# ymxlzgy/echoscene

Measured on AMD Instinct MI355X. Metric: denoising steps/sec (layout+SDF) for 32-node scene-graph, 64^3 SDF (3x16^3 latent), full step = one DDPM layout step + one DDIM shape step over all objects; `value` = the FUSED step (both loops as one hipGraph per step, the layout step on a parallel branch: what the K timed steps ran); `full_steps_p, higher is better.
Workload: dtype f16 MFMA operands / f32 accumulate (shape UNet); f32 (layout, GCN)

## Files before the change

### echoscene_amd/csrc/es_vol.hip

```cpp
#include "es_common.h"
#include <string>
#include <algorithm>
#include <cstdlib>
#include <mutex>
#include <type_traits>

namespace {

__device__ __forceinline__ int f_swz(int row) { return (0x1320 >> (((row >> 2) & 3) * 4)) & 3; }

constexpr int GN_VT = 64;

__global__ __launch_bounds__(256) void k_gn_partial(const es_gn_args a, float* part, int vt) {
    __shared__ float ssum4[4][2048], ssq4[4][2048];
    float* ssum = ssum4[0];
    float* ssq = ssq4[0];
    const int o = blockIdx.y, tile = blockIdx.x, C = a.C1 + a.C2;
    const int v0 = tile * vt;
    const int nv = min(vt, a.V - v0);
    const int c4n = C >> 2;
    const int CX = 64;
    const int cx = threadIdx.x & (CX - 1), vy = threadIdx.x >> 6;
    for (int c4 = cx; c4 < c4n; c4 += CX) {
        const int c = c4 * 4;
// ... 1578 lines not shown
    f4 fin[MI2][7];
#pragma unroll
    for (int i2 = 0; i2 < MI2; ++i2)
#pragma unroll
        for (int j = 0; j < 7; ++j) {
            const int i = strm * MI2 + i2;
            f4 v = ((const f4*)smem)[(long)(0 * NCH_ + hh) * (PART_FLOATS / 4) + (i * 7 + j) * 64 + lane];
#pragma unroll
            for (int s = 1; s < KS_; ++s) v += ((const f4*)smem)[(long)(s * NCH_ + hh) * (PART_FLOATS / 4) + (i * 7 + j) * 64 + lane];
            fin[i2][j] = v;
        }
    asm volatile("s_waitcnt lgkmcnt(0)" ::: "memory");
    if constexpr (NCH_ == 1) conv_epilogue<64, 8, true, true, EPI_>(a, g, fin, smem, M, m0, by * BN + half0 * 112, 2 * wave, lane, S, bz, ncdhw);
    else conv_epilogue<64, 4, true, true, EPI_>(a, g, fin, smem, M, m0, by * BN, wave, lane, S, bz, ncdhw);
}

template <int EPI_, int NS_ = 3>
__global__ __launch_bounds__(768, 3) void k_linear_ws(const es_conv_args a, const ConvGeom g, int ncb) {
    constexpr int BM_ = 256, NC_ = 8, NP_ = 4, NS = NS_;
    constexpr int WROWS = BM_ / (NC_ / 2), MI = WROWS / 16;
    constexpr int A_BYTES = BM_ * BK * 2, B_BYTES = BNP * BK * 2, STAGE_BYTES = A_BYTES + B_BYTES, RING_BYTES = NS * STAGE_BYTES;
    constexpr int NA = (BM_ / 16) / NP_, NB = (BNP / 16) / NP_, NLOAD = NA + NB;
    constexpr unsigned OOB = 0x80000000u;
    typedef __attribute__((address_space(3))) void* lds_ptr;
    extern __shared__ __attribute__((aligned(16))) char smem[];
    const int tid = threadIdx.x, lane = tid & 63;
    const int wave = __builtin_amdgcn_readfirstlane(tid >> 6);
    const long M = (long)g.O * g.D * g.H * g.W;
#ifdef ES_STAMP
    unsigned long long* stamp = g_stamp_buf ? g_stamp_buf + ((size_t)(blockIdx.x + gridDim.x * blockIdx.y) * (NC_ + NP_) + wave) * 8 : nullptr;
#endif
    ES_STAMP_AT(0);
    int bx, byg;
    {
        const int gx = gridDim.x, gy = gridDim.y, nwg = gx * gy;
        const int orig = blockIdx.x + gx * blockIdx.y;
        const int xcd = orig & 7, q = nwg >> 3, r = nwg & 7;
        const int L = (xcd < r ? xcd * (q + 1) : r * (q + 1) + (xcd - r) * q) + (orig >> 3);
        const long slab = (long)a.Cin * BN * 2 * ncb;
        int npanel = (int)(((long)gy * slab + (3L << 20) - 1) / (3L << 20));
        npanel = npanel < 1 ? 1 : (npanel > gy ? gy : npanel);
        const int Pw = (gy + npanel - 1) / npanel, full = gx * Pw;
        const int p = L / full, rr = L - p * full;
        const int w = (gy - p * Pw) < Pw ? (gy - p * Pw) : Pw;
        bx = rr / w;
        byg = p * Pw + (rr - bx * w);
    }
    const long m0 = (long)bx * BM_;
    const int by0 = byg * ncb;
    const int kch = a.Cin >> 5;
    const int total = kch * ncb;
    if (wave >= NC_) {
        const int pw = wave - NC_;
        unsigned voff[NA];
#pragma unroll
        for (int j = 0; j < NA; ++j) {
            const int p = (pw + NP_ * j) * 64 + lane;
            const int row = p >> 2;
            const long m = m0 + row;
            voff[j] = m < M ? (unsigned)(m * a.Cin * 2 + (((p & 3) ^ f_swz(row)) * 16)) : OOB;
        }
        const __amdgpu_buffer_rsrc_t rA = __builtin_amdgcn_make_buffer_rsrc(uniform_ptr(a.a), (short)0, (int)OOB, 0x00020000);
        const _Float16* Wg = (const _Float16*)a.w;
        int cb = 0, c = 0, islot = 0;
        __amdgpu_buffer_rsrc_t rB = __builtin_amdgcn_make_buffer_rsrc(uniform_ptr(Wg + (long)by0 * kch * (BNP * BK)), (short)0, (int)OOB, 0x00020000);
        const unsigned voffB = (unsigned)lane * 16u;
        auto issue = [&]() __attribute__((always_inline)) {
            char* dst = smem + __builtin_amdgcn_readfirstlane(islot) * STAGE_BYTES;
            const unsigned sA = (unsigned)__builtin_amdgcn_readfirstlane(c) * 64u;
            const unsigned sB = (unsigned)__builtin_amdgcn_readfirstlane(c) * (unsigned)B_BYTES;
#pragma unroll
            for (int j = 0; j < NA; ++j)
                __builtin_amdgcn_raw_ptr_buffer_load_lds(rA, (lds_ptr)(dst + (pw + NP_ * j) * 1024), 16, (int)voff[j], (int)sA, 0, 0);
#pragma unroll
            for (int j = 0; j < NB; ++j) {
                const int q = pw + NP_ * j;
                const unsigned vB = q * 16 >= BN ? OOB : voffB;
                __builtin_amdgcn_raw_ptr_buffer_load_lds(rB, (lds_ptr)(dst + A_BYTES + q * 1024), 16, (int)vB, (int)(sB + (unsigned)q * 1024u), 0, 0);
            }
            islot = islot == NS - 1 ? 0 : islot + 1;
            if (++c == kch) {
                c = 0; ++cb;
                rB = __builtin_amdgcn_make_buffer_rsrc(uniform_ptr(Wg + (long)(by0 + cb) * kch * (BNP * BK)), (short)0, (int)OOB, 0x00020000);
            }
        };
        issue();
        if (total > 1) issue();
        if (NS == 4 && total > 2) issue();
        for (int u = 0; u < total; ++u) {
            const int ahead = total - 1 - u < NS - 2 ? total - 1 - u : NS - 2;
            if (ahead >= 2) wait_vmcnt<2 * NLOAD>(); else if (ahead == 1) wait_vmcnt<NLOAD>(); else wait_vmcnt<0>();
            __builtin_amdgcn_s_barrier();
            if (u + NS - 1 < total) issue();
        }
        return;
    }
    const int wm = wave >> 1, wn = wave & 1;
    const int i16 = lane & 15, q = lane >> 4;
    const int fragA = (wm * WROWS + i16) * 64 + ((q ^ f_swz(i16)) << 4);
    const int fragB = A_BYTES + (wn * 112 + i16) * 64 + ((q ^ f_swz(i16)) << 4);
    int slot = 0;
    for (int cb = 0; cb < ncb; ++cb) {
        f4 acc[MI][7];
#pragma unroll
        for (int i = 0; i < MI; ++i)
#pragma unroll
            for (int j = 0; j < 7; ++j) acc[i][j] = f4{0.f, 0.f, 0.f, 0.f};
        h8 af[MI], bfr[7];
        __builtin_amdgcn_s_barrier();
        ws_read_frags<MI>(smem + slot * STAGE_BYTES, fragA, fragB, af, bfr);
        slot = slot == NS - 1 ? 0 : slot + 1;
        for (int ks = 0; ks + 1 < kch; ++ks) {
            const char* const An = smem + slot * STAGE_BYTES;
            slot = slot == NS - 1 ? 0 : slot + 1;
#pragma unroll
            for (int j = 0; j < 7; ++j) acc[0][j] = __builtin_amdgcn_mfma_f32_16x16x32_f16(af[0], bfr[j], acc[0][j], 0, 0, 0);
            __builtin_amdgcn_sched_barrier(0);
            asm volatile("s_waitcnt lgkmcnt(0)" ::: "memory");
            __builtin_amdgcn_s_barrier();
            __builtin_amdgcn_sched_barrier(0);
#pragma unroll
            for (int i = 1; i < MI; ++i) {
                af[i - 1] = *(const h8*)(An + fragA + (i - 1) * 1024);
                __builtin_amdgcn_sched_barrier(0);
                if (i < MI - 1) {
#pragma unroll
                    for (int j = 0; j < 7; ++j) acc[i][j] = __builtin_amdgcn_mfma_f32_16x16x32_f16(af[i], bfr[j], acc[i][j], 0, 0, 0);
                    __builtin_amdgcn_sched_barrier(0);
                } else {
#pragma unroll
                    for (int j = 0; j < 7; ++j) {
                        acc[i][j] = __builtin_amdgcn_mfma_f32_16x16x32_f16(af[i], bfr[j], acc[i][j], 0, 0, 0);
                        __builtin_amdgcn_sched_barrier(0);
                        bfr[j] = *(const h8*)(An + fragB + j * 1024);
                        __builtin_amdgcn_sched_barrier(0);
                    }
                }
            }
            af[MI - 1] = *(const h8*)(An + fragA + (MI - 1) * 1024);
            __builtin_amdgcn_sched_barrier(0);
        }
        ws_mma<MI>(acc, af, bfr);
#ifdef ES_STAMP
        if (cb < 3) ES_STAMP_AT(1 + 2 * cb);
#endif
        conv_epilogue<BM_, NC_, true, true, EPI_, true>(a, g, acc, smem + RING_BYTES, M, m0, (by0 + cb) * BN, wave, lane, 1, 0, 0);
#ifdef ES_STAMP
        if (cb < 3) ES_STAMP_AT(2 + 2 * cb);
#endif
    }
}

constexpr int AT_K = 64;

template <int DP, int NWV, int NRT, int MINW = (DP <= 64 ? 3 : 2)>
__global__ __launch_bounds__(64 * NWV, MINW) void k_attention(const es_attn_args a) {
    constexpr int AT_Q = 16 * NRT * NWV;
    constexpr int KLD = DP + 8;
    __shared__ __attribute__((aligned(16))) _Float16 Ks[AT_K * KLD];
    __shared__ __attribute__((aligned(16))) _Float16 Vs[AT_K * KLD];
    const int tid = threadIdx.x, lane = tid & 63, wave = tid >> 6;
    const int i16 = lane & 15, q4 = lane >> 4;
    const int nx = gridDim.x, nwg = nx * (int)gridDim.y;
    const int orig = blockIdx.x + nx * blockIdx.y;
    const int xcd = orig & 7, xq = nwg >> 3, xr = nwg & 7;
    const int L = (xcd < xr ? xcd * (xq + 1) : xr * (xq + 1) + (xcd - xr) * xq) + (orig >> 3);
    const int bh = L / nx, rtile = L - bh * nx;
    const int b = bh / a.heads, h = bh - b * a.heads;
    const int C = a.heads * a.dhead, ldq = 3 * C;
    const _Float16* base = (const _Float16*)a.qkv + (long)b * a.Ntok * ldq + h * a.dhead;
    const int q0 = rtile * AT_Q + wave * (16 * NRT);

    h8 qf[NRT][DP / 32];
#pragma unroll
    for (int rt = 0; rt < NRT; ++rt)
#pragma unroll
        for (int kc = 0; kc < DP / 32; ++kc) {
            const int d0 = kc * 32 + q4 * 8, row = q0 + rt * 16 + i16;
            const _Float16* p = base + (long)row * ldq + d0;
#pragma unroll
            for (int e = 0; e < 8; ++e) qf[rt][kc][e] = (d0 + e < a.dhead && row < a.Ntok) ? p[e] : (_Float16)0.f;
        }
    f4 oacc[NRT][DP / 16];
    float mrow[NRT], lrow[NRT];
#pragma unroll
    for (int rt = 0; rt < NRT; ++rt) {
        mrow[rt] = -INFINITY; lrow[rt] = 0.f;
#pragma unroll
        for (int j = 0; j < DP / 16; ++j) oacc[rt][j] = f4{0.f, 0.f, 0.f, 0.f};
    }

    constexpr int NT = 64 * NWV, CPR = DP / 4, NITEM = AT_K * CPR, NIT = (NITEM + NT - 1) / NT;
    constexpr bool PREFETCH = DP <= 96;
    h4 kreg[NIT], vreg[NIT];
    unsigned kvoff[NIT];
#pragma unroll
    for (int it = 0; it < NIT; ++it) {
        const int idx = tid + it * NT;
        const int key = idx / CPR, d = (idx - key * CPR) * 4;
        kvoff[it] = (idx < NITEM && d < a.dhead) ? (unsigned)(key * ldq + d) * 2u : 0x80000000u;
    }
    const int nrec = (int)(((long)(a.Ntok - 1) * ldq + a.dhead) * 2);
    const __amdgpu_buffer_rsrc_t rK = __builtin_amdgcn_make_buffer_rsrc(uniform_ptr(base + C), (short)0, nrec, 0x00020000);
    const __amdgpu_buffer_rsrc_t rV = __builtin_amdgcn_make_buffer_rsrc(uniform_ptr(base + 2 * C), (short)0, nrec, 0x00020000);
    auto gload = [&](int k0) __attribute__((always_inline)) {
        const unsigned koff = (unsigned)k0 * (unsigned)ldq * 2u;
#pragma unroll
        for (int it = 0; it < NIT; ++it) {
            kreg[it] = __builtin_bit_cast(h4, __builtin_amdgcn_raw_buffer_load_b64(rK, (int)(kvoff[it] + koff), 0, 0));
            vreg[it] = __builtin_bit_cast(h4, __builtin_amdgcn_raw_buffer_load_b64(rV, (int)(kvoff[it] + koff), 0, 0));
        }
    };
    if (PREFETCH) gload(0);
    for (int k0 = 0; k0 < a.Ntok; k0 += AT_K) {
        __syncthreads();
#pragma unroll
        for (int it = 0; it < NIT; ++it) {
            const int idx = tid + it * NT;
            if (idx < NITEM) {
                const int key = idx / CPR, d = (idx - key * CPR) * 4;
                h4 kv = kreg[PREFETCH ? it : 0], vv = vreg[PREFETCH ? it : 0];
                if (!PREFETCH) {
                    kv = h4{0, 0, 0, 0}; vv = h4{0, 0, 0, 0};
                    if (d < a.dhead && k0 + key < a.Ntok) {
                        const _Float16* p = base + (long)(k0 + key) * ldq + d;
                        kv = *(const h4*)(p + C);
                        vv = *(const h4*)(p + 2 * C);
                    }
                }
                *(h4*)&Ks[key * KLD + d] = kv;
                *(h4*)&Vs[key * KLD + d] = vv;
            }
        }
        __syncthreads();
        if (PREFETCH && k0 + AT_K < a.Ntok) gload(k0 + AT_K);
        f4 s[NRT][4];
#pragma unroll
        for (int rt = 0; rt < NRT; ++rt)
#pragma unroll
            for (int t = 0; t < 4; ++t) s[rt][t] = f4{0.f, 0.f, 0.f, 0.f};
#pragma unroll
        for (int t = 0; t < 4; ++t)
#pragma unroll
            for (int kc = 0; kc < DP / 32; ++kc) {
                const h8 kf = *(const h8*)&Ks[(t * 16 + i16) * KLD + kc * 32 + q4 * 8];
#pragma unroll
                for (int rt = 0; rt < NRT; ++rt) s[rt][t] = __builtin_amdgcn_mfma_f32_16x16x32_f16(kf, qf[rt][kc], s[rt][t], 0, 0, 0);
            }
        h8 pf[NRT][2];
        typedef float f2 __attribute__((ext_vector_type(2)));
        const float c2 = a.scale * 1.44269504088896340736f;
        if (k0 + AT_K > a.Ntok) {
            asm volatile("" ::: "memory");
#pragma unroll
            for (int rt = 0; rt < NRT; ++rt)
#pragma unroll
                for (int t = 0; t < 4; ++t)
#pragma unroll
                    for (int r = 0; r < 4; ++r) {
                        float v = k0 + t * 16 + q4 * 4 + r >= a.Ntok ? -INFINITY : s[rt][t][r];
                        asm volatile("" : "+v"(v));
                        s[rt][t][r] = v;
                    }
        }
#pragma unroll
        for (int rt = 0; rt < NRT; ++rt) {
            float mx = -INFINITY;
#pragma unroll
            for (int t = 0; t < 4; ++t)
#pragma unroll
                for (int r = 0; r < 4; ++r) mx = fmaxf(mx, s[rt][t][r]);
            {
                float e, o;
                es_pair16(mx, e, o); mx = fmaxf(e, o);
                es_pair32(mx, e, o); mx = fmaxf(e, o);
            }
            const float mnew = fmaxf(mrow[rt], mx * c2);
            const float alpha = __builtin_amdgcn_exp2f(mrow[rt] - mnew);
            const f2 c22 = {c2, c2}, nm2 = {-mnew, -mnew};
            f2 ps2 = {0.f, 0.f};
#pragma unroll
            for (int t = 0; t < 4; ++t)
#pragma unroll
                for (int hf = 0; hf < 2; ++hf) {
                    const f2 v = {s[rt][t][2 * hf], s[rt][t][2 * hf + 1]};
                    const f2 e = __builtin_elementwise_fma(v, c22, nm2);
                    const f2 pp = {__builtin_amdgcn_exp2f(e[0]), __builtin_amdgcn_exp2f(e[1])};
                    ps2 += pp;
                    pf[rt][t >> 1][(t & 1) * 4 + 2 * hf] = (_Float16)pp[0];
                    pf[rt][t >> 1][(t & 1) * 4 + 2 * hf + 1] = (_Float16)pp[1];
                }
            float ps = ps2[0] + ps2[1];
            {
                float e, o;
                es_pair16(ps, e, o); ps = e + o;
                es_pair32(ps, e, o); ps = e + o;
            }
            lrow[rt] = lrow[rt] * alpha + ps;
            mrow[rt] = mnew;
            if (__ballot(alpha != 1.0f) != 0) {
                const f2 al2 = {alpha, alpha};
#pragma unroll
                for (int j = 0; j < DP / 16; ++j) {
                    f2 lo = {oacc[rt][j][0], oacc[rt][j][1]}, hi = {oacc[rt][j][2], oacc[rt][j][3]};
                    lo *= al2; hi *= al2;
                    oacc[rt][j] = f4{lo[0], lo[1], hi[0], hi[1]};
                }
            }
        }
#pragma unroll
        for (int kc = 0; kc < AT_K / 32; ++kc)
#pragma unroll
            for (int j = 0; j < DP / 16; ++j) {
                typedef short s4v __attribute__((ext_vector_type(4)));
                typedef __attribute__((address_space(3))) s4v* lds_s4;
                const _Float16* vp = &Vs[(kc * 32 + q4 * 4 + (i16 >> 2)) * KLD + j * 16 + (i16 & 3) * 4];
                const h4 v0 = __builtin_bit_cast(h4, __builtin_amdgcn_ds_read_tr16_b64_v4i16((lds_s4)vp));
                const h4 v1 = __builtin_bit_cast(h4, __builtin_amdgcn_ds_read_tr16_b64_v4i16((lds_s4)(vp + 16 * KLD)));
                const h8 vf = {v0[0], v0[1], v0[2], v0[3], v1[0], v1[1], v1[2], v1[3]};
#pragma unroll
                for (int rt = 0; rt < NRT; ++rt) oacc[rt][j] = __builtin_amdgcn_mfma_f32_16x16x32_f16(vf, pf[rt][kc], oacc[rt][j], 0, 0, 0);
            }
    }
    _Float16* out = (_Float16*)a.out_f16 + (long)b * a.Ntok * C + h * a.dhead;
#pragma unroll
    for (int rt = 0; rt < NRT; ++rt) {
        const int row = q0 + rt * 16 + i16;
        if (row >= a.Ntok) continue;
        const float inv = 1.0f / lrow[rt];
#pragma unroll
        for (int j = 0; j < DP / 16; ++j) {
            const int d = j * 16 + q4 * 4;
            if (d < a.dhead) {
                const f4 o = oacc[rt][j] * inv;
                const h4 hv = {(_Float16)o[0], (_Float16)o[1], (_Float16)o[2], (_Float16)o[3]};
                *(h4*)&out[(long)row * C + d] = hv;
            }
        }
    }
}

__global__ __launch_bounds__(256) void k_conv_small_n(const es_conv_args a, const ConvGeom g, int ncdhw) {
    extern __shared__ __attribute__((aligned(16))) char smem[];
    _Float16* wl = (_Float16*)smem;
    const int wn = a.N * 27 * a.Cin;
    for (int i = threadIdx.x * 8; i < wn; i += 256 * 8) *(h8*)(wl + i) = *(const h8*)((const _Float16*)a.w + i);
    __syncthreads();
    const long M = (long)g.O * g.D * g.H * g.W;
    const long m = (long)blockIdx.x * 256 + threadIdx.x;
    if (m >= M) return;
    const int w_ = (int)(m & (g.W - 1)), h_ = (int)((m >> g.lw) & (g.H - 1)), d_ = (int)((m >> (g.lw + g.lh)) & (g.D - 1));
    const long o = m >> (g.lw + g.lh + g.ld);
    float acc[4] = {0.f, 0.f, 0.f, 0.f};
    const _Float16* A = (const _Float16*)a.a;
    for (int tap = 0; tap < 27; ++tap) {
        const int id = d_ + tap / 9 - 1, ih = h_ + (tap / 3) % 3 - 1, iw = w_ + tap % 3 - 1;
        if (id < 0 || id >= g.D || ih < 0 || ih >= g.H || iw < 0 || iw >= g.W) continue;
        const _Float16* src = A + (((o * g.D + id) * g.H + ih) * g.W + iw) * a.Cin;
        for (int c = 0; c < a.Cin; c += 8) {
            const h8 x = *(const h8*)(src + c);
#pragma unroll
            for (int n = 0; n < 4; ++n) {
                if (n < a.N) {
                    const h8 wv = *(const h8*)(wl + (n * 27 + tap) * a.Cin + c);
#pragma unroll
                    for (int e = 0; e < 8; ++e) acc[n] += (float)x[e] * (float)wv[e];
                }
            }
        }
    }
    const long V = (long)g.D * g.H * g.W;
    for (int n = 0; n < a.N; ++n) {
        float v = acc[n] + (a.bias ? a.bias[n] : 0.f);
        if (ncdhw) a.out_f32[(o * a.N + n) * V + (m - o * V)] = v;
        else a.out_f32[m * a.out_ld + n] = v;
    }
}

__global__ __launch_bounds__(256) void k_conv_small_n_tiled(const es_conv_args a, const ConvGeom g, int ncdhw) {
    extern __shared__ __attribute__((aligned(16))) char smem[];
    const int Cin = a.Cin, c8n = Cin >> 3, vstride = Cin * 2 + 16;
    char* xt = smem;
    _Float16* wl = (_Float16*)(smem + 1000 * vstride);
    const int wn = a.N * 27 * Cin;
    for (int i = threadIdx.x * 8; i < wn; i += 256 * 8) *(h8*)(wl + i) = *(const h8*)((const _Float16*)a.w + i);
    const int tw = g.W >> 3, th = g.H >> 3, td = g.D >> 3;
    int t = blockIdx.x;
    const int bw = t % tw; t /= tw;
    const int bh = t % th; t /= th;
    const int bd = t % td;
    const long o = t / td;
    const _Float16* A = (const _Float16*)a.a + o * (long)g.D * g.H * g.W * Cin;
    for (int i = threadIdx.x; i < 1000 * c8n; i += 256) {
        const int c8 = i % c8n, v = i / c8n;
        const int lw = v % 10, lh = (v / 10) % 10, ld_ = v / 100;
        const int iw = bw * 8 + lw - 1, ih = bh * 8 + lh - 1, id = bd * 8 + ld_ - 1;
        h8 x = {0, 0, 0, 0, 0, 0, 0, 0};
        if (iw >= 0 && iw < g.W && ih >= 0 && ih < g.H && id >= 0 && id < g.D)
            x = *(const h8*)(A + (((long)id * g.H + ih) * g.W + iw) * Cin + c8 * 8);
        *(h8*)(xt + v * vstride + c8 * 16) = x;
    }
    __syncthreads();
    typedef _Float16 h2v __attribute__((ext_vector_type(2)));
    float acc[2][4] = {{0.f, 0.f, 0.f, 0.f}, {0.f, 0.f, 0.f, 0.f}};
    const int lw = threadIdx.x & 7, lh = (threadIdx.x >> 3) & 7, ld0 = threadIdx.x >> 6;
    for (int tap = 0; tap < 27; ++tap) {
        const int kd = tap / 9, kh = (tap / 3) % 3, kw = tap % 3;
        const char* p0 = xt + (((ld0 + kd) * 10 + lh + kh) * 10 + lw + kw) * vstride;
        const char* p1 = p0 + 400 * vstride;
        for (int c8 = 0; c8 < c8n; ++c8) {
            const h8 x0 = *(const h8*)(p0 + c8 * 16), x1 = *(const h8*)(p1 + c8 * 16);
#pragma unroll
            for (int n = 0; n < 4; ++n) {
                if (n < a.N) {
                    const h8 wv = *(const h8*)(wl + (n * 27 + tap) * Cin + c8 * 8);
#pragma unroll
                    for (int e = 0; e < 4; ++e) {
                        const h2v w2 = {wv[2 * e], wv[2 * e + 1]};
                        acc[0][n] = __builtin_amdgcn_fdot2(h2v{x0[2 * e], x0[2 * e + 1]}, w2, acc[0][n], false);
                        acc[1][n] = __builtin_amdgcn_fdot2(h2v{x1[2 * e], x1[2 * e + 1]}, w2, acc[1][n], false);
                    }
                }
            }
        }
    }
    const long V = (long)g.D * g.H * g.W;
#pragma unroll
    for (int k = 0; k < 2; ++k) {
        const long vox = (((long)(bd * 8 + ld0 + 4 * k) * g.H) + bh * 8 + lh) * g.W + bw * 8 + lw;
        for (int n = 0; n < a.N; ++n) {
            const float v = acc[k][n] + (a.bias ? a.bias[n] : 0.f);
            if (ncdhw) a.out_f32[(o * a.N + n) * V + vox] = v;
            else a.out_f32[(o * V + vox) * a.out_ld + n] = v;
        }
    }
}

constexpr int N16_ROWS = 6 * 6 * 18;
constexpr int N16_A_BYTES = 44 * 1024, N16_B_BYTES = 28 * 1024;

__global__ __launch_bounds__(256, 2) void k_conv_n16(const es_conv_args a, const ConvGeom g) {
    typedef __attribute__((address_space(3))) void* lds_ptr;
    constexpr unsigned OOB = 0x80000000u;
    extern __shared__ __attribute__((aligned(16))) char smem[];
    char* As = smem;
    char* Bs = smem + N16_A_BYTES;
    const int tid = threadIdx.x, lane = tid & 63;
    const int wave = __builtin_amdgcn_readfirstlane(tid >> 6);
    const int tw = g.W >> 4, th = g.H >> 2, td = g.D >> 2;
    int t = blockIdx.x;
    const int bw = t % tw; t /= tw;
    const int bh = t % th; t /= th;
    const int bd = t % td;
    const int o = t / td;
    const int Cin = a.Cin, kch = Cin >> 5;
    constexpr int NPA = 11, NPB = 7;
    unsigned voff[NPA];
#pragma unroll
    for (int j = 0; j < NPA; ++j) {
        const int piece = wave + 4 * j;
        const int slot = piece * 64 + lane;
        const int row = slot >> 2;
        const int lc = (slot & 3) ^ f_swz(row);
        const int hw = row % 18, hh = (row / 18) % 6, hd = row / 108;
        const int d = bd * 4 - 1 + hd, h = bh * 4 - 1 + hh, w = bw * 16 - 1 + hw;
        const bool ok = row < N16_ROWS && d >= 0 && d < g.D && h >= 0 && h < g.H && w >= 0 && w < g.W;
        voff[j] = ok ? (unsigned)((((o * g.D + d) * g.H + h) * g.W + w) * Cin * 2 + lc * 16) : OOB;
    }
    const __amdgpu_buffer_rsrc_t rA = __builtin_amdgcn_make_buffer_rsrc(uniform_ptr(a.a), (short)0, (int)OOB, 0x00020000);
    const __amdgpu_buffer_rsrc_t rB = __builtin_amdgcn_make_buffer_rsrc(uniform_ptr(a.w), (short)0, (int)OOB, 0x00020000);
    const int i16 = lane & 15, q = lane >> 4;
    const int rowbase = (wave * 6) * 18 + i16;
    f4 acc[4];
#pragma unroll
    for (int i = 0; i < 4; ++i) acc[i] = f4{0.f, 0.f, 0.f, 0.f};
// ... 678 lines not shown
        const int np = vo("conv_st_np");
        const dim3 grid((unsigned)((M + st_bm - 1) / st_bm), ntn, S);
        const bool stt = want_stats && epi_stats;
        int rc = 1;
        const int ns = vo("conv_st_ns");
        if (st_bm == 64 && np == 4 && ns == 3) rc = launch_ws<64, 4, 4, 3>(a, g, ncdhw, grid, st, upm, geglu, stt);
        else if (st_bm == 64 && np == 4 && ns == 6) rc = launch_ws<64, 4, 4, 6>(a, g, ncdhw, grid, st, upm, geglu, stt);
        else if (st_bm == 128 && np == 4 && ns == 3) rc = launch_ws<128, 4, 4, 3>(a, g, ncdhw, grid, st, upm, geglu, stt);
        else if (st_bm == 128 && np == 8 && ns == 3) rc = launch_ws<128, 4, 8, 3>(a, g, ncdhw, grid, st, upm, geglu, stt);
        else if (st_bm == 128 && np == 8 && ns == 5) rc = launch_ws<128, 4, 8, 5>(a, g, ncdhw, grid, st, upm, geglu, stt);
        else ES_REQUIRE(false, "es_conv_mfma_f16: conv_st_bm=%d conv_st_np=%d conv_st_ns=%d is not a built tile", st_bm, np, ns);
        if (rc) return rc;
        stats_done = stt;
    } else if (deep) {
        S = 1;
        hipLaunchKernelGGL(k_linear_deep, dim3((unsigned)((M + 63) / 64), ntn, 1), dim3(256), 7 * (64 * BK * 2 + BNP * BK * 2), st, *a, g);
    } else if (route256) {
        dim3 grid((unsigned)((M + 255) / 256), ntn, S);
        if (ncb > 1) {
            const dim3 lgrid(grid.x, (unsigned)(ntn / ncb), 1);
            constexpr int LDSLIN = LDS256 + 8 * 16 * 116 * 4;
            static const char* ring_env = getenv("ES_LIN_RING");
            if (geglu && ring_env && atoi(ring_env) == 4) hipLaunchKernelGGL((k_linear_ws<ES_EPI_GEGLU, 4>), lgrid, dim3(768), LDSLIN_GEGLU, st, *a, g, ncb);
            else if (geglu) hipLaunchKernelGGL((k_linear_ws<ES_EPI_GEGLU>), lgrid, dim3(768), LDSLIN, st, *a, g, ncb);
            else hipLaunchKernelGGL((k_linear_ws<ES_EPI_NONE>), lgrid, dim3(768), LDSLIN, st, *a, g, ncb);
        } else if (ws && (!geglu || !upm)) {
            static const char* ns_env = getenv("ES_CONV_NS");
            const int ns = ns_env ? atoi(ns_env) : 3;
            const bool stt = want_stats && epi_stats;
            static const char* a3_env = getenv("ES_CONV_A3");
            const bool a3 = (a3_env ? atoi(a3_env) != 0 : ES_CONV_A3_DEFAULT) && a->taps == 27 && a->mode == ES_CONV_SAME && !a->a2 && a->W <= 16 && a->W >= 4;
            if (a3) {
                static std::once_flag once3;
                static hipError_t err3 = hipSuccess;
                std::call_once(once3, [] {
                    err3 = hipFuncSetAttribute((const void*)k_conv_ws3<false>, hipFuncAttributeMaxDynamicSharedMemorySize, 6 * 16384);
                    for (auto fl : {std::pair<const void*, int>{(const void*)k_conv_ws3<true>, 6 * 16384}, {(const void*)k_conv_ws3<false, true>, 9 * 16384},
                                    {(const void*)k_conv_ws3<true, true>, 9 * 16384}}) {
                        const hipError_t e2 = hipFuncSetAttribute(fl.first, hipFuncAttributeMaxDynamicSharedMemorySize, fl.second);
                        if (err3 == hipSuccess) err3 = e2;
                    }
                });
                static const char* gb_env = getenv("ES_CONV_GB");
                ES_REQUIRE(err3 == hipSuccess, "es_conv_mfma_f16: hipFuncSetAttribute failed: %s", hipGetErrorString(err3));
                if (!gb_env || atoi(gb_env) != 0) {
                    if (stt) hipLaunchKernelGGL((k_conv_ws3<true, true>), grid, dim3(768), 9 * 16384, st, *a, g);
                    else hipLaunchKernelGGL((k_conv_ws3<false, true>), grid, dim3(768), 9 * 16384, st, *a, g);
                }
                else if (stt) hipLaunchKernelGGL((k_conv_ws3<true>), grid, dim3(768), 6 * 16384, st, *a, g);
                else hipLaunchKernelGGL((k_conv_ws3<false>), grid, dim3(768), 6 * 16384, st, *a, g);
                if (stt) stats_done = true;
            } else {
            int rc;
            if (ns == 4) rc = launch_ws<256, 8, 4, 4>(a, g, ncdhw, grid, st, upm, geglu, stt);
            else if (ns == 5) rc = launch_ws<256, 8, 4, 5>(a, g, ncdhw, grid, st, upm, geglu, stt);
            else rc = launch_ws<256, 8, 4, 3>(a, g, ncdhw, grid, st, upm, geglu, stt);
            if (rc) return rc;
            if (stt) stats_done = true;
            }
        }
        else if (upm) hipLaunchKernelGGL((k_conv_lean<256, 8, true>), grid, dim3(512), LDS256, st, *a, g, ncdhw);
        else hipLaunchKernelGGL((k_conv_lean<256, 8>), grid, dim3(512), LDS256, st, *a, g, ncdhw);
    } else if ((wg128 >= 512 || S > 1) && !tiny_split) {
        dim3 grid((unsigned)((M + 127) / 128), ntn, S);
        if (upm) hipLaunchKernelGGL((k_conv_lean<128, 4, true>), grid, dim3(256), LDS128, st, *a, g, ncdhw);
        else hipLaunchKernelGGL((k_conv_lean<128, 4>), grid, dim3(256), LDS128, st, *a, g, ncdhw);
    } else {
        dim3 grid((unsigned)((M + 63) / 64), ntn, tiny_split ? S : 1);
        if (upm) hipLaunchKernelGGL((k_conv_lean<64, 4, true>), grid, dim3(256), LDS64, st, *a, g, ncdhw);
        else hipLaunchKernelGGL((k_conv_lean<64, 4>), grid, dim3(256), LDS64, st, *a, g, ncdhw);
    }
    if (S > 1) {
        const long n4 = M * (a->N / 4);
        const int blocks = (int)((n4 + 255) / 256 < 4096 ? (n4 + 255) / 256 : 4096);
        if (a->gn_part_out && part_ok) {
            const int V = a->D * a->H * a->W;
            const int vt = gn_voxel_tile(Oh, V);
            hipLaunchKernelGGL(k_conv_splitk_reduce_gn, dim3((V + vt - 1) / vt, a->O), dim3(256), 0, st, *a, M, V, S, vt);
        } else
            hipLaunchKernelGGL(k_conv_splitk_reduce, dim3(blocks), dim3(256), 0, st, *a, M, a->D * a->H * a->W, S);
    }
    if (want_stats && !stats_done) {
        ES_REQUIRE(a->out_f32, "es_conv_mfma_f16: this launch's route forms gn_stats_out by a pass over the fp32 output: out_f32 must be given "
                               "(es_conv_emits_gn_stats() == 0)");
        const long n4 = ((M + 63) / 64) * (a->N / 4);
        const int blocks = (int)((n4 + 255) / 256 < 8192 ? (n4 + 255) / 256 : 8192);
        hipLaunchKernelGGL(k_rowgroup_stats, dim3(blocks), dim3(256), 0, st, (const float*)a->out_f32, M, a->N, a->out_ld, a->gn_stats_out);
    }
    ES_CHECK_HIP(hipGetLastError());
    return 0;
}

extern "C" int es_conv_mfma_f16(const es_conv_args* a, es_stream stream) { return conv_dispatch(a, stream, nullptr); }

extern "C" int es_conv_emits_gn_stats(const es_conv_args* a) {
    int e = 0;
    return conv_dispatch(a, nullptr, &e) == 0 ? (e & 1) : -1;
}

extern "C" int es_conv_emits_gn_part(const es_conv_args* a) {
    int e = 0;
    return conv_dispatch(a, nullptr, &e) == 0 ? ((e >> 1) & 1) : -1;
}

extern "C" int es_conv_split_of(const es_conv_args* a) {
    int e = 0;
    return conv_dispatch(a, nullptr, &e) == 0 ? (e >> 8) : -1;
}

extern "C" int es_groupnorm_vol(const es_gn_args* a, es_stream stream) {
    const int C = a->C1 + a->C2;
    ES_REQUIRE(C % a->groups == 0 && C <= 2048 && a->groups <= 64, "es_groupnorm_vol: C=%d groups=%d", C, a->groups);
    ES_REQUIRE(a->C1 % 8 == 0 && a->C2 % 8 == 0, "es_groupnorm_vol: channel counts must be multiples of 8 (%d,%d)", a->C1, a->C2);
    ES_REQUIRE(a->stats != nullptr, "es_groupnorm_vol: stats scratch missing");
    const long Oh = a->O_hint < 0 ? -(long)a->O_hint : (long)(a->O_hint > a->O ? a->O_hint : a->O);
    const int vt = gn_voxel_tile(Oh, a->V);
    const int ntiles = (a->V + vt - 1) / vt;
    float* part = a->stats;
    const bool from_rg = a->stats1 && (!a->x2 || a->stats2) && a->V % 64 == 0 && (a->x1_is_f16 || vo("gn_rg") != 0);
    ES_REQUIRE(!a->x1_is_f16 || (from_rg && !a->x2 && !a->raw_f16),
               "es_groupnorm_vol: an f16 source needs the producer's row-group sums (stats1), one source, no raw copy");
    ES_REQUIRE(!a->part_in || (!from_rg && !a->x2), "es_groupnorm_vol: part_in needs one source and no row-group sums");
    if (a->part_in) part = (float*)a->part_in;
    else if (!from_rg) hipLaunchKernelGGL(k_gn_partial, dim3(ntiles, a->O), dim3(256), 0, (hipStream_t)stream, *a, part, vt);
    int vpb = 32;
    while (vpb > 8 && (long)a->O * ((a->V + vpb - 1) / vpb) < 512) vpb >>= 1;
    while (vpb < 1024 && (long)a->O * ((a->V + vpb - 1) / vpb) > 16384) vpb <<= 1;
    const float* fin = nullptr;
    if (from_rg) {
        hipLaunchKernelGGL(k_gn_finalize_rg, dim3(a->groups, a->O), dim3(256), 0, (hipStream_t)stream, *a, part);
        fin = part;
    } else if (ntiles > 128) {
        float* f = a->part_in ? a->stats : part + (size_t)a->O * ntiles * a->groups * 2;
        hipLaunchKernelGGL(k_gn_finalize, dim3(a->groups, a->O), dim3(256), 0, (hipStream_t)stream, *a, part, ntiles, f);
        fin = f;
    }
    hipLaunchKernelGGL(k_gn_apply, dim3((a->V + vpb - 1) / vpb, a->O), dim3(256), 0, (hipStream_t)stream, *a, part, ntiles, vpb, fin);
    ES_CHECK_HIP(hipGetLastError());
    return 0;
}

extern "C" int es_layernorm_tokens(const es_ln_args* a, es_stream stream) {
    ES_REQUIRE(a->C <= 1024 && a->C > 0 && a->C % 4 == 0, "es_layernorm_tokens: C=%d (a multiple of 4, max 1024)", a->C);
    long wgs = ((long)a->M + 3) / 4;
    if (wgs > 2048) wgs = 2048;
    hipLaunchKernelGGL(k_layernorm, dim3((unsigned)wgs), dim3(256), 0, (hipStream_t)stream, *a);
    ES_CHECK_HIP(hipGetLastError());
    return 0;
}

extern "C" int es_attention_f16(const es_attn_args* a, es_stream stream) {
    ES_REQUIRE(a->dhead % 4 == 0 && a->dhead <= 256 && a->dhead > 0, "es_attention_f16: dhead=%d (multiple of 4, <= 256)", a->dhead);
    ES_REQUIRE(a->scale > 0.f, "es_attention_f16: scale=%g must be positive (the row maximum is taken over the raw scores)", (double)a->scale);
    const bool big = a->Ntok >= 512 && a->dhead <= 96;
    const int rows = big ? 128 : 64;
    dim3 grid((a->Ntok + rows - 1) / rows, a->B * a->heads);
    hipStream_t st = (hipStream_t)stream;
    if (a->dhead <= 32) { if (big) hipLaunchKernelGGL((k_attention<32, 4, 2>), grid, dim3(256), 0, st, *a); else hipLaunchKernelGGL((k_attention<32, 4, 1>), grid, dim3(256), 0, st, *a); }
    else if (a->dhead <= 64) { if (big) hipLaunchKernelGGL((k_attention<64, 4, 2>), grid, dim3(256), 0, st, *a); else hipLaunchKernelGGL((k_attention<64, 4, 1>), grid, dim3(256), 0, st, *a); }
    else if (a->dhead <= 96) { if (big) hipLaunchKernelGGL((k_attention<96, 4, 2>), grid, dim3(256), 0, st, *a); else hipLaunchKernelGGL((k_attention<96, 4, 1>), grid, dim3(256), 0, st, *a); }
    else hipLaunchKernelGGL((k_attention<256, 4, 1>), grid, dim3(256), 0, st, *a);
    ES_CHECK_HIP(hipGetLastError());
    return 0;
}

extern "C" int es_geglu_f16(const es_geglu_args* a, es_stream stream) {
    ES_REQUIRE(a->C4 % 4 == 0, "es_geglu_f16: C4=%d", a->C4);
    const long n4 = (long)a->M * (a->C4 / 4);
    const int blocks = (int)((n4 + 255) / 256 < 8192 ? (n4 + 255) / 256 : 8192);
    hipLaunchKernelGGL(k_geglu, dim3(blocks), dim3(256), 0, (hipStream_t)stream, *a);
    ES_CHECK_HIP(hipGetLastError());
    return 0;
}

static int latent_to_cl(const float* x, int O, int C, int V, int Cpad, void* out, int is_f32, es_stream stream) {
    const long n = (long)O * V * Cpad;
    const int blocks = (int)((n + 255) / 256 < 4096 ? (n + 255) / 256 : 4096);
    hipLaunchKernelGGL(k_to_cl, dim3(blocks), dim3(256), 0, (hipStream_t)stream, x, O, C, V, Cpad, (_Float16*)out, is_f32);
    ES_CHECK_HIP(hipGetLastError());
    return 0;
}
extern "C" int es_latent_to_cl_f16(const float* x, int O, int C, int V, int Cpad, void* out, es_stream stream) { return latent_to_cl(x, O, C, V, Cpad, out, 0, stream); }
extern "C" int es_latent_to_cl_f32(const float* x, int O, int C, int V, int Cpad, void* out, es_stream stream) { return latent_to_cl(x, O, C, V, Cpad, out, 1, stream); }

extern "C" int es_split_f16x3(const float* x, long M, int C, void* out, es_stream stream) {
    ES_REQUIRE(x && out && M > 0 && C > 0 && C % 4 == 0, "es_split_f16x3: M=%ld C=%d (C a multiple of 4)", M, C);
    const long n = M * (C / 4);
    const int blocks = (int)((n + 255) / 256 < 8192 ? (n + 255) / 256 : 8192);
    hipLaunchKernelGGL(k_split_f16x3, dim3(blocks), dim3(256), 0, (hipStream_t)stream, x, M, C, (_Float16*)out);
    ES_CHECK_HIP(hipGetLastError());
    return 0;
}

extern "C" int es_shape_stem(const es_stem_args* a, es_stream stream) {
    const long n1 = (long)a->O * 32 * 512, n2 = (long)a->O * 512;
    const int Cx = a->Cin ? a->Cin : 3;
    ES_REQUIRE(Cx >= 1 && Cx <= 4, "es_shape_stem: Cin=%d (3 or 4)", Cx);
    (void)n1;
    hipLaunchKernelGGL(k_stem1, dim3(64, a->O), dim3(256), (size_t)(Cx * 288 + 32 * Cx * 27) * 4, (hipStream_t)stream, *a);
    {
        static std::once_flag once_s;
        static hipError_t attr_s = hipSuccess;
        std::call_once(once_s, [] { attr_s = hipFuncSetAttribute((const void*)k_stem2, hipFuncAttributeMaxDynamicSharedMemorySize, 32 * 513 * 4); });
        ES_REQUIRE(attr_s == hipSuccess, "es_shape_stem: hipFuncSetAttribute failed: %s", hipGetErrorString(attr_s));
    }
    hipLaunchKernelGGL(k_stem2, dim3((unsigned)((n2 * 8 + 255) / 256)), dim3(256), 32 * 513 * 4, (hipStream_t)stream, *a);
    ES_CHECK_HIP(hipGetLastError());
    return 0;
}

extern "C" int es_vq_lookup(const es_vq_args* a, es_stream stream) {
    ES_REQUIRE(a->n_embed > 0 && a->n_embed * 16 <= 160 * 1024 - 1024, "es_vq_lookup: n_embed=%d too large for LDS", a->n_embed);
    ES_REQUIRE(a->Cpad >= 3, "es_vq_lookup: Cpad=%d", a->Cpad);
    {
        static std::once_flag once;
        static hipError_t attr_err = hipSuccess;
        std::call_once(once, [] {
            attr_err = hipFuncSetAttribute((const void*)k_vq_lookup, hipFuncAttributeMaxDynamicSharedMemorySize, 160 * 1024 - 1024);
        });
        ES_REQUIRE(attr_err == hipSuccess, "es_vq_lookup: hipFuncSetAttribute failed: %s", hipGetErrorString(attr_err));
    }
    const long M = (long)a->O * a->V;
    hipLaunchKernelGGL(k_vq_lookup, dim3((unsigned)((M + 255) / 256)), dim3(256), (size_t)a->n_embed * 16, (hipStream_t)stream, *a);
    ES_CHECK_HIP(hipGetLastError());
    return 0;
}
```

Measured before the change: 55.84.

## Defer softmax rescale with threshold, fold row-sum into PV MFMA, split ragged tile

```diff
diff --git a/echoscene_amd/csrc/es_vol.hip b/echoscene_amd/csrc/es_vol.hip
--- a/echoscene_amd/csrc/es_vol.hip
+++ b/echoscene_amd/csrc/es_vol.hip
@@ -1754,8 +1754,9 @@
 }
 
 constexpr int AT_K = 64;
-
-template <int DP, int NWV, int NRT, int MINW = (DP <= 64 ? 3 : 2)>
+constexpr float AT_TAU = 8.f;
+
+template <int DP, int NWV, int NRT, bool LSUM, int MINW = (DP <= 64 ? 3 : 2)>
 __global__ __launch_bounds__(64 * NWV, MINW) void k_attention(const es_attn_args a) {
     constexpr int AT_Q = 16 * NRT * NWV;
     constexpr int KLD = DP + 8;
@@ -1796,12 +1797,15 @@
     constexpr bool PREFETCH = DP <= 96;
     h4 kreg[NIT], vreg[NIT];
     unsigned kvoff[NIT];
+    int vsoff[NIT];
 #pragma unroll
     for (int it = 0; it < NIT; ++it) {
         const int idx = tid + it * NT;
         const int key = idx / CPR, d = (idx - key * CPR) * 4;
         kvoff[it] = (idx < NITEM && d < a.dhead) ? (unsigned)(key * ldq + d) * 2u : 0x80000000u;
-    }
+        vsoff[it] = key * KLD + ((LSUM && d == a.dhead) ? DP : d);
+    }
+    if (LSUM && tid < AT_K) *(h4*)&Vs[tid * KLD + a.dhead] = h4{(_Float16)1.f, (_Float16)0.f, (_Float16)0.f, (_Float16)0.f};
     const int nrec = (int)(((long)(a.Ntok - 1) * ldq + a.dhead) * 2);
     const __amdgpu_buffer_rsrc_t rK = __builtin_amdgcn_make_buffer_rsrc(uniform_ptr(base + C), (short)0, nrec, 0x00020000);
     const __amdgpu_buffer_rsrc_t rV = __builtin_amdgcn_make_buffer_rsrc(uniform_ptr(base + 2 * C), (short)0, nrec, 0x00020000);
@@ -1814,7 +1818,8 @@
         }
     };
     if (PREFETCH) gload(0);
-    for (int k0 = 0; k0 < a.Ntok; k0 += AT_K) {
+    auto tile = [&](const int k0, auto ragged_c) __attribute__((always_inline)) {
+        constexpr bool RAGGED = decltype(ragged_c)::value;
         __syncthreads();
 #pragma unroll
         for (int it = 0; it < NIT; ++it) {
@@ -1831,40 +1836,41 @@
                     }
                 }
                 *(h4*)&Ks[key * KLD + d] = kv;
-                *(h4*)&Vs[key * KLD + d] = vv;
+                *(h4*)&Vs[vsoff[it]] = vv;
             }
         }
         __syncthreads();
         if (PREFETCH && k0 + AT_K < a.Ntok) gload(k0 + AT_K);
         f4 s[NRT][4];
+        h8 kf[NRT > 1 ? 4 : 1][DP / 32];
+        if (NRT > 1)
+#pragma unroll
+            for (int t = 0; t < 4; ++t)
+#pragma unroll
+                for (int kc = 0; kc < DP / 32; ++kc) kf[NRT > 1 ? t : 0][kc] = *(const h8*)&Ks[(t * 16 + i16) * KLD + kc * 32 + q4 * 8];
 #pragma unroll
         for (int rt = 0; rt < NRT; ++rt)
 #pragma unroll
-            for (int t = 0; t < 4; ++t) s[rt][t] = f4{0.f, 0.f, 0.f, 0.f};
-#pragma unroll
-        for (int t = 0; t < 4; ++t)
-#pragma unroll
-            for (int kc = 0; kc < DP / 32; ++kc) {
-                const h8 kf = *(const h8*)&Ks[(t * 16 + i16) * KLD + kc * 32 + q4 * 8];
-#pragma unroll
-                for (int rt = 0; rt < NRT; ++rt) s[rt][t] = __builtin_amdgcn_mfma_f32_16x16x32_f16(kf, qf[rt][kc], s[rt][t], 0, 0, 0);
+            for (int t = 0; t < 4; ++t) {
+                s[rt][t] = f4{0.f, 0.f, 0.f, 0.f};
+#pragma unroll
+                for (int kc = 0; kc < DP / 32; ++kc) {
+                    const h8 k8 = NRT > 1 ? kf[NRT > 1 ? t : 0][kc] : *(const h8*)&Ks[(t * 16 + i16) * KLD + kc * 32 + q4 * 8];
+                    s[rt][t] = __builtin_amdgcn_mfma_f32_16x16x32_f16(k8, qf[rt][kc], s[rt][t], 0, 0, 0);
+                }
             }
         h8 pf[NRT][2];
-        typedef float f2 __attribute__((ext_vector_type(2)));
         const float c2 = a.scale * 1.44269504088896340736f;
-        if (k0 + AT_K > a.Ntok) {
-            asm volatile("" ::: "memory");
+        if (RAGGED) {
 #pragma unroll
             for (int rt = 0; rt < NRT; ++rt)
 #pragma unroll
                 for (int t = 0; t < 4; ++t)
 #pragma unroll
-                    for (int r = 0; r < 4; ++r) {
-                        float v = k0 + t * 16 + q4 * 4 + r >= a.Ntok ? -INFINITY : s[rt][t][r];
-                        asm volatile("" : "+v"(v));
-                        s[rt][t][r] = v;
-                    }
-        }
+                    for (int r = 0; r < 4; ++r) s[rt][t][r] = k0 + t * 16 + q4 * 4 + r >= a.Ntok ? -INFINITY : s[rt][t][r];
+        }
+        float mref[NRT], psum[NRT];
+        bool moved = false;
 #pragma unroll
         for (int rt = 0; rt < NRT; ++rt) {
             float mx = -INFINITY;
@@ -1877,39 +1883,45 @@
                 es_pair16(mx, e, o); mx = fmaxf(e, o);
                 es_pair32(mx, e, o); mx = fmaxf(e, o);
             }
-            const float mnew = fmaxf(mrow[rt], mx * c2);
-            const float alpha = __builtin_amdgcn_exp2f(mrow[rt] - mnew);
-            const f2 c22 = {c2, c2}, nm2 = {-mnew, -mnew};
-            f2 ps2 = {0.f, 0.f};
+            const float mt = mx * c2;
+            const bool up = mt > mrow[rt] + AT_TAU;
+            moved |= up;
+            mref[rt] = up ? mt : mrow[rt];
+            const float nm = -mref[rt];
+            float ps = 0.f;
 #pragma unroll
             for (int t = 0; t < 4; ++t)
 #pragma unroll
-                for (int hf = 0; hf < 2; ++hf) {
-                    const f2 v = {s[rt][t][2 * hf], s[rt][t][2 * hf + 1]};
-                    const f2 e = __builtin_elementwise_fma(v, c22, nm2);
-                    const f2 pp = {__builtin_amdgcn_exp2f(e[0]), __builtin_amdgcn_exp2f(e[1])};
-                    ps2 += pp;
-                    pf[rt][t >> 1][(t & 1) * 4 + 2 * hf] = (_Float16)pp[0];
-                    pf[rt][t >> 1][(t & 1) * 4 + 2 * hf + 1] = (_Float16)pp[1];
+                for (int r = 0; r < 4; r += 2) {
+                    float p0 = __builtin_amdgcn_exp2f(__builtin_fmaf(s[rt][t][r], c2, nm));
+                    float p1 = __builtin_amdgcn_exp2f(__builtin_fmaf(s[rt][t][r + 1], c2, nm));
+                    asm("" : "+v"(p0), "+v"(p1));
+                    if (!LSUM) ps += p0 + p1;
+                    pf[rt][t >> 1][(t & 1) * 4 + r] = (_Float16)p0;
+                    pf[rt][t >> 1][(t & 1) * 4 + r + 1] = (_Float16)p1;
                 }
-            float ps = ps2[0] + ps2[1];
-            {
+            if (!LSUM) {
                 float e, o;
                 es_pair16(ps, e, o); ps = e + o;
                 es_pair32(ps, e, o); ps = e + o;
             }
-            lrow[rt] = lrow[rt] * alpha + ps;
-            mrow[rt] = mnew;
-            if (__ballot(alpha != 1.0f) != 0) {
-                const f2 al2 = {alpha, alpha};
-#pragma unroll
-                for (int j = 0; j < DP / 16; ++j) {
-                    f2 lo = {oacc[rt][j][0], oacc[rt][j][1]}, hi = {oacc[rt][j][2], oacc[rt][j][3]};
-                    lo *= al2; hi *= al2;
-                    oacc[rt][j] = f4{lo[0], lo[1], hi[0], hi[1]};
-                }
-            }
-        }
+            psum[rt] = ps;
+        }
+        if (__ballot(moved) != 0) {
+#pragma unroll
+            for (int rt = 0; rt < NRT; ++rt) {
+                const float alpha = __builtin_amdgcn_exp2f(mrow[rt] - mref[rt]);
+#pragma unroll
+                for (int j = 0; j < DP / 16; ++j)
+#pragma unroll
+                    for (int r = 0; r < 4; ++r) oacc[rt][j][r] *= alpha;
+                if (!LSUM) lrow[rt] *= alpha;
+                mrow[rt] = mref[rt];
+            }
+        }
+        if (!LSUM)
+#pragma unroll
+            for (int rt = 0; rt < NRT; ++rt) lrow[rt] += psum[rt];
 #pragma unroll
         for (int kc = 0; kc < AT_K / 32; ++kc)
 #pragma unroll
@@ -1923,6 +1935,19 @@
 #pragma unroll
                 for (int rt = 0; rt < NRT; ++rt) oacc[rt][j] = __builtin_amdgcn_mfma_f32_16x16x32_f16(vf, pf[rt][kc], oacc[rt][j], 0, 0, 0);
             }
+    };
+    int k0 = 0;
+    for (; k0 + AT_K <= a.Ntok; k0 += AT_K) tile(k0, std::false_type{});
+    if (k0 < a.Ntok) tile(k0, std::true_type{});
+    if (LSUM) {
+        const int jl = a.dhead >> 4, src = i16 + 16 * ((a.dhead & 15) >> 2);
+#pragma unroll
+        for (int rt = 0; rt < NRT; ++rt) {
+            float v = 0.f;
+#pragma unroll
+            for (int j = 0; j < DP / 16; ++j) v = j == jl ? oacc[rt][j][0] : v;
+            lrow[rt] = __shfl(v, src);
+        }
     }
     _Float16* out = (_Float16*)a.out_f16 + (long)b * a.Ntok * C + h * a.dhead;
 #pragma unroll
@@ -2907,14 +2932,23 @@
 extern "C" int es_attention_f16(const es_attn_args* a, es_stream stream) {
     ES_REQUIRE(a->dhead % 4 == 0 && a->dhead <= 256 && a->dhead > 0, "es_attention_f16: dhead=%d (multiple of 4, <= 256)", a->dhead);
     ES_REQUIRE(a->scale > 0.f, "es_attention_f16: scale=%g must be positive (the row maximum is taken over the raw scores)", (double)a->scale);
-    const bool big = a->Ntok >= 512 && a->dhead <= 96;
+    const bool big = a->Ntok >= 256 && a->dhead <= 96;
     const int rows = big ? 128 : 64;
     dim3 grid((a->Ntok + rows - 1) / rows, a->B * a->heads);
     hipStream_t st = (hipStream_t)stream;
-    if (a->dhead <= 32) { if (big) hipLaunchKernelGGL((k_attention<32, 4, 2>), grid, dim3(256), 0, st, *a); else hipLaunchKernelGGL((k_attention<32, 4, 1>), grid, dim3(256), 0, st, *a); }
-    else if (a->dhead <= 64) { if (big) hipLaunchKernelGGL((k_attention<64, 4, 2>), grid, dim3(256), 0, st, *a); else hipLaunchKernelGGL((k_attention<64, 4, 1>), grid, dim3(256), 0, st, *a); }
-    else if (a->dhead <= 96) { if (big) hipLaunchKernelGGL((k_attention<96, 4, 2>), grid, dim3(256), 0, st, *a); else hipLaunchKernelGGL((k_attention<96, 4, 1>), grid, dim3(256), 0, st, *a); }
-    else hipLaunchKernelGGL((k_attention<256, 4, 1>), grid, dim3(256), 0, st, *a);
+#define ES_ATTN_LAUNCH(DP_)                                                                                                         \
+    do {                                                                                                                            \
+        const bool ls = a->dhead < DP_;                                                                                             \
+        if (big) { if (ls) hipLaunchKernelGGL((k_attention<DP_, 4, 2, true>), grid, dim3(256), 0, st, *a);                          \
+                   else hipLaunchKernelGGL((k_attention<DP_, 4, 2, false>), grid, dim3(256), 0, st, *a); }                           \
+        else { if (ls) hipLaunchKernelGGL((k_attention<DP_, 4, 1, true>), grid, dim3(256), 0, st, *a);                              \
+               else hipLaunchKernelGGL((k_attention<DP_, 4, 1, false>), grid, dim3(256), 0, st, *a); }                               \
+    } while (0)
+    if (a->dhead <= 32) ES_ATTN_LAUNCH(32);
+    else if (a->dhead <= 64) ES_ATTN_LAUNCH(64);
+    else if (a->dhead <= 96) ES_ATTN_LAUNCH(96);
+    else hipLaunchKernelGGL((k_attention<256, 4, 1, false>), grid, dim3(256), 0, st, *a);
+#undef ES_ATTN_LAUNCH
     ES_CHECK_HIP(hipGetLastError());
     return 0;
 }
```

Result: no change. 55.85, median of 6 (+0.0%).
